# Foxhead-Studio/InsTaG

Measured on AMD Instinct MI355X. Metric: train-step frames/sec @512x512, 100k Gaussians, higher is better.
Workload: dtype f32; 1 GPU; C3: train_face step, 100k Gaussians + 6 grid encodes + UMF/PMF motion nets (DeepSpeech feats), 512x512, SH degree 1, image + attention map in one raster pass, L1+DSSIM, Adam; targets = uniform noise (SURVEY 8d); gaussians=100000, sh_degree=1, parallelism=dp1, ranks_reported_by_backend=1, execution=hipGraph replay, timing=one window of 1714 steps after 5 warm-up steps

## Files before the change

instag_amd/_lib.py:

```python
from __future__ import annotations

import ctypes as C
import os
import threading

from . import _cabi

HERE = os.path.dirname(os.path.abspath(__file__))
LIB_PATH = os.path.join(HERE, "lib", "libinstag_hip.so")

_lib = None
_lock = threading.Lock()

vp = C.c_void_p
i32 = C.c_int32
f32 = C.c_float

_STRUCTS, _PROTOTYPES, _CONSTANTS = _cabi.read()
globals().update((cls.__name__, cls) for cls in _STRUCTS.values())
EXPORTED_SYMBOLS = tuple(_PROTOTYPES)
ABI_VERSION = _CONSTANTS["INSTAG_ABI_VERSION"]
E_ARG = _CONSTANTS["INSTAG_E_ARG"]
FACE_LOSS = {k[len("INSTAG_FACE_LOSS_"):]: v for k, v in _CONSTANTS.items() if k.startswith("INSTAG_FACE_LOSS_")}

_WAV2VEC_STRUCTS, _WAV2VEC_PROTOTYPES, WAV2VEC = _cabi.read(os.path.join(os.path.dirname(_cabi.HEADER), "instag_wav2vec.h"))
globals().update((cls.__name__, cls) for cls in _WAV2VEC_STRUCTS.values())

_HUBERT_STRUCTS, _HUBERT_PROTOTYPES, HUBERT = _cabi.read(os.path.join(os.path.dirname(_cabi.HEADER), "instag_hubert.h"),
                                                         _WAV2VEC_STRUCTS)

_, _FRAME_CODE_WIDE_PROTOTYPES, _ = _cabi.read(os.path.join(os.path.dirname(_cabi.HEADER), "instag_frame_code_wide.h"))

_DEEPSPEECH_STRUCTS, _DEEPSPEECH_PROTOTYPES, DEEPSPEECH = _cabi.read(os.path.join(os.path.dirname(_cabi.HEADER),
                                                                              "instag_deepspeech.h"))
globals().update((cls.__name__, cls) for cls in _DEEPSPEECH_STRUCTS.values())

_LANDMARKS_STRUCTS, _LANDMARKS_PROTOTYPES, LANDMARKS = _cabi.read(os.path.join(os.path.dirname(_cabi.HEADER),
                                                                             "instag_landmarks.h"))
globals().update((cls.__name__, cls) for cls in _LANDMARKS_STRUCTS.values())

_FACE_DETECT_STRUCTS, _FACE_DETECT_PROTOTYPES, FACE_DETECT = _cabi.read(os.path.join(os.path.dirname(_cabi.HEADER),
                                                                                   "instag_face_detect.h"))
globals().update((cls.__name__, cls) for cls in _FACE_DETECT_STRUCTS.values())


_STREAMS = {}


def side_stream(device, tag, priority=0):
    import torch
    device = torch.device(device)
    index = device.index if device.index is not None else torch.cuda.current_device()
    key = (index, tag)
    s = _STREAMS.get(key)
    if s is None:
        taken = {v.cuda_stream for (d, _), v in _STREAMS.items() if d == index}
        for _ in range(64):
            s = torch.cuda.Stream(device=torch.device("cuda", index), priority=priority)
            if s.cuda_stream not in taken:
                break
        else:
            raise RuntimeError(f"no distinct HIP stream left for {tag!r} ({len(taken)} in use on device {index})")
        _STREAMS[key] = s
    return s


def capture_stream(device=None):
    import torch
    if device is None:
        device = torch.device("cuda", torch.cuda.current_device())
    return side_stream(device, "capture", priority=-1)


def warmup_stream(device):
    return side_stream(device, "warmup")

# ... 59 lines not shown


def may_fork(device=None) -> bool:
    import torch
    if _LEAF_STREAMS and any(torch.cuda.current_stream(device) == s for s in _LEAF_STREAMS):
        return False
    if not torch.cuda.is_current_stream_capturing():
        return True
    return _CAPTURE_ORIGIN is not None and torch.cuda.current_stream(device) == _CAPTURE_ORIGIN


_LEAF_STREAMS = []


def leaf_stream(stream):
    if all(stream != s for s in _LEAF_STREAMS):
        _LEAF_STREAMS.append(stream)


def lib():
    global _lib
    if _lib is not None:
        return _lib
    with _lock:
        if _lib is not None:
            return _lib
        if not os.path.exists(LIB_PATH):
            from . import build as _build
            _build.build(verbose=False)
        import torch
        handle = C.CDLL(LIB_PATH)
        for name, (res, args) in {**_PROTOTYPES, **_WAV2VEC_PROTOTYPES, **_HUBERT_PROTOTYPES,
                                  **_FRAME_CODE_WIDE_PROTOTYPES, **_DEEPSPEECH_PROTOTYPES,
                                  **_LANDMARKS_PROTOTYPES, **_FACE_DETECT_PROTOTYPES}.items():
            if not hasattr(handle, name):
                raise RuntimeError(f"{LIB_PATH} does not export {name}: rebuild it (python -m instag_amd.build)")
            fn = getattr(handle, name)
            fn.restype = res
            fn.argtypes = args
        if handle.instag_abi_version() != ABI_VERSION:
            raise RuntimeError(f"{LIB_PATH} has ABI version {handle.instag_abi_version()}, the bindings expect "
                               f"{ABI_VERSION}: rebuild it (python -c 'import __graft_entry__ as g; g.build()')")
        _lib = handle
    return _lib


def check(code: int, what: str = ""):
    if code != 0:
        msg = lib().instag_last_error().decode("utf-8", "replace")
        raise RuntimeError(f"{what}: {msg}" if what else msg)


def check_arg(code: int, what: str):
    if code != 0:
        msg = lib().instag_last_error().decode("utf-8", "replace")
        raise (ValueError if code == E_ARG else RuntimeError)(f"{what}: {msg}")


def workspace_bytes(nbytes: int) -> int:
    if nbytes == 0:
        raise ValueError(lib().instag_last_error().decode("utf-8", "replace"))
    return int(nbytes)


def ptr(t):
    return None if t is None else C.c_void_p(t.data_ptr())

# ... 5 lines not shown
```

instag_amd/csrc/raster_api.hip:

```cpp
#include <cstdio>
#include <cstdlib>
#include <cstring>

#include <mutex>
#include <vector>

#include "raster_internal.hpp"

namespace instag {

static thread_local std::string g_err;
void set_error(const std::string& msg) { g_err = msg; }

namespace {
struct ProfState {
  std::mutex mu;
  int mask = 0;
  struct Pair { hipEvent_t a, b; };
  std::vector<Pair> pending[INSTAG_PROF_KERNELS];
  double total_ms[INSTAG_PROF_KERNELS] = {0};
  int64_t launches[INSTAG_PROF_KERNELS] = {0};
  struct GraphPair { hipEvent_t a = nullptr, b = nullptr; int kernel = -1; bool closed = false; };
  std::vector<GraphPair> graph_pool;
  int graph_used = 0;
};
ProfState& prof() { static ProfState p; return p; }
}

static hipError_t record_external(hipEvent_t ev, hipStream_t stream) {
  static bool direct_ok = true;
  if (direct_ok) {
    if (hipEventRecordWithFlags(ev, stream, hipEventRecordExternal) == hipSuccess) return hipSuccess;
    (void)hipGetLastError();
    direct_ok = false;
  }
  hipStreamCaptureStatus st = hipStreamCaptureStatusNone;
  unsigned long long id = 0;
  hipGraph_t graph = nullptr;
  const hipGraphNode_t* deps = nullptr;
// ... 127 lines not shown
  L.tile_partials = o; o = align_up(o + (size_t)L.pre_blocks * WIDE_DIGITS * sizeof(uint32_t), 256);
  L.total = o;
  return L;
}

ImageLayout image_layout(int32_t H, int32_t W) {
  ImageLayout L;
  const size_t tiles = (size_t)div_up(W, TILE_X) * div_up(H, TILE_Y);
  const size_t P = (size_t)H * W;
  size_t o = 0;
  L.ranges = o; o = align_up(o + tiles * 2 * sizeof(int32_t), 256);
  L.n_contrib = o; o = align_up(o + P * sizeof(uint32_t), 256);
  L.final_T = o; o = align_up(o + P * sizeof(float), 256);
  L.tile_rounds = o; o = align_up(o + tiles * sizeof(uint32_t), 256);
  L.blend_mode = o; o = align_up(o + sizeof(uint32_t), 256);
  L.total = o;
  return L;
}

BinningLayout binning_layout(int64_t R, int32_t H, int32_t W) {
  BinningLayout L;
  const size_t r = (size_t)(R > 0 ? R : 1);
  const size_t tiles = (size_t)div_up(W, TILE_X) * div_up(H, TILE_Y);
  size_t o = 0;
  L.keys_unsorted = o; o = align_up(o + r * sizeof(uint32_t), 256);
  L.vals_unsorted = o; o = align_up(o + r * sizeof(uint32_t), 256);
  L.keys = o; o = align_up(o + r * sizeof(uint32_t), 256);
  L.vals = o; o = align_up(o + r * sizeof(uint32_t), 256);
  L.ktmp = o; o = align_up(o + r * sizeof(uint32_t), 256);
  L.vtmp = o; o = align_up(o + r * sizeof(uint32_t), 256);
  L.gid_unsorted = o; o = align_up(o + r * sizeof(uint32_t), 256);
  L.point_list = o; o = align_up(o + r * sizeof(uint32_t), 256);
  L.tsort_blocks = sort_blocks((uint32_t)r, SORT_IPT_TILE);
  const size_t wide_words = wide_tiles((int)tiles) ? (size_t)tile_pass_blocks((uint32_t)r) * 2 * ((tiles + 1) / 2) : 0;
  const size_t sort_words = 16 + std::max((size_t)3 * L.tsort_blocks * 256, wide_words);
  L.row_flag_stride = align_up(r, 16);
  L.seg_slots = r / SEG_LEN + tiles + 2;
  L.tsort_zero_words = sort_words + 4 + 2 * L.row_flag_stride / 4 + 8 * tiles + L.seg_slots;
  L.tsort_zero = o;
  L.seg_count = o + sort_words * sizeof(uint32_t);
  L.row_flag = L.seg_count + 4 * sizeof(uint32_t);
  L.fwd_sync = L.row_flag + 2 * L.row_flag_stride;
  L.seg_flag = L.fwd_sync + 8 * tiles * sizeof(uint32_t);
  o = align_up(o + L.tsort_zero_words * sizeof(uint32_t), 256);
  L.tsort_digit_base = o; o = align_up(o + (size_t)HIST_SLICES * 3 * 256 * sizeof(uint32_t), 256);
  L.tsort_partials = o; o = align_up(o + (size_t)1024 * 3 * 256 * sizeof(uint32_t), 256);
  L.sort_count = o; o = align_up(o + sizeof(uint32_t), 256);
  L.seg_queue = o; o = align_up(o + 2 * L.seg_slots * sizeof(uint32_t), 256);
  L.seg_state = o; o = align_up(o + L.seg_slots * SEG_FLOATS * TILE_PIX * sizeof(float), 256);
  L.total = o;
  return L;
}

static int validate(const instag_raster_args* a) {
  INSTAG_REQUIRE(a != nullptr, "raster args is NULL");
  INSTAG_REQUIRE(a->N >= 0, "N must be >= 0");
  INSTAG_REQUIRE(a->image_height > 0 && a->image_width > 0, "image size must be positive");
  INSTAG_REQUIRE(a->image_height <= 16368 && a->image_width <= 16368, "image larger than 16368 px not supported");
  INSTAG_REQUIRE((a->shs != nullptr) != (a->colors_precomp != nullptr),
                 "Please provide excatly one of either SHs or precomputed colors!");
  INSTAG_REQUIRE(((a->scales != nullptr && a->rotations != nullptr) && a->cov3Ds_precomp == nullptr) ||
                     ((a->scales == nullptr && a->rotations == nullptr) && a->cov3Ds_precomp != nullptr),
                 "Please provide exactly one of either scale/rotation pair or precomputed 3D covariance!");
  INSTAG_REQUIRE(a->E == 0 || a->E == 1, "extra_attrs: only 0 or 1 channel is supported");
  INSTAG_REQUIRE(a->sh_degree >= 0 && a->sh_degree <= 3, "sh_degree must be in [0,3]");
  if (a->shs) INSTAG_REQUIRE((a->sh_degree + 1) * (a->sh_degree + 1) <= a->M, "shs has fewer coefficients than sh_degree needs");
  INSTAG_REQUIRE(a->shs_rest == nullptr || (a->shs != nullptr && a->M >= 2), "shs_rest needs shs (the DC term) and M >= 2");
// ... 386 lines not shown
  const size_t n = std::min<size_t>((size_t)max_pairs, BL.seg_slots);
  if (n > 0) INSTAG_CHECK_HIP(hipMemcpyAsync(pairs, bb + BL.seg_queue, n * 2 * sizeof(uint32_t), hipMemcpyDeviceToDevice, s));
  if (blend_mode)
    INSTAG_CHECK_HIP(hipMemcpyAsync(blend_mode, ib + IL.blend_mode, sizeof(uint32_t), hipMemcpyDeviceToDevice, s));
  return INSTAG_OK;
}

int instag_raster_debug_export_flags(const void* geom, size_t geom_bytes, int32_t N, uint32_t* flags,
                                     instag_stream_t stream_) {
  const GeomLayout GL = geom_layout(N);
  INSTAG_REQUIRE(geom != nullptr && flags != nullptr, "debug_export_flags: NULL pointer");
  if (geom_bytes < GL.total) { set_error("geom buffer too small"); return INSTAG_E_SPACE; }
  if (N > 0)
    INSTAG_CHECK_HIP(hipMemcpyAsync(flags, (const char*)geom + GL.flags, (size_t)N * 4, hipMemcpyDeviceToDevice,
                                    (hipStream_t)stream_));
  return INSTAG_OK;
}

int instag_debug_depth_sort(const instag_raster_args* a, void* geom, size_t geom_bytes, uint64_t* stamps,
                            uint32_t* order_out, instag_stream_t stream_) {
  INSTAG_REQUIRE(a != nullptr && a->N > 0, "debug_depth_sort: N must be positive");
  const GeomLayout L = geom_layout(a->N);
  if (geom_bytes < L.total) { set_error("geom buffer too small"); return INSTAG_E_SPACE; }
  const Camera c = make_camera(a);
  if (int e = depth_sort(c, a, (char*)geom, L, (hipStream_t)stream_, stamps)) return e;
  if (order_out)
    INSTAG_CHECK_HIP(hipMemcpyAsync(order_out, (char*)geom + L.order, (size_t)a->N * 4, hipMemcpyDeviceToDevice,
                                    (hipStream_t)stream_));
  return INSTAG_OK;
}

uint32_t instag_debug_depth_sort_blocks(int32_t N) { return geom_layout(N).dsort_blocks; }

int instag_raster_sort_stalls(uint32_t* count, int32_t synchronize, instag_stream_t stream_) {
  INSTAG_REQUIRE(count != nullptr, "sort_stalls: count is NULL");
  return read_sort_stalls(count, (hipStream_t)stream_, synchronize != 0);
}

int instag_raster_sort_stalls_clear(instag_stream_t stream_) { return clear_sort_stalls((hipStream_t)stream_); }

int instag_debug_scan_stall_probe(instag_stream_t stream_) {
  hipStream_t s = (hipStream_t)stream_;
  constexpr int N = 8;
  uint32_t host[3 * N];
  for (int i = 0; i < N; ++i) { host[i] = (uint32_t)i; host[N + i] = 1u; host[2 * N + i] = 0u; }
  const uint64_t state_host[4] = {1ull, 0ull, 0ull, 0ull};
  char* dev = nullptr;
  INSTAG_CHECK_HIP(hipMalloc((void**)&dev, sizeof(host) + sizeof(state_host)));
  hipError_t err = hipMemcpyAsync(dev, host, sizeof(host), hipMemcpyHostToDevice, s);
  if (err == hipSuccess) err = hipMemcpyAsync(dev + sizeof(host), state_host, sizeof(state_host), hipMemcpyHostToDevice, s);
  int rc = INSTAG_OK;
  if (err == hipSuccess)
    rc = launch_scan_counts(N, (const uint32_t*)dev, (const uint32_t*)dev + N, (uint32_t*)dev + 2 * N,
                            (uint64_t*)(dev + sizeof(host)), s);
  if (err == hipSuccess) err = hipStreamSynchronize(s);
  (void)hipFree(dev);
  if (err != hipSuccess) { set_error(std::string("scan_stall_probe: ") + hipGetErrorString(err)); return INSTAG_E_HIP; }
  return rc;
}

int instag_prof_enable(int mask) {
  ProfState& p = prof();
  std::lock_guard<std::mutex> lk(p.mu);
  p.mask = mask;
  return INSTAG_OK;
}
// ... 92 lines not shown
```

instag_amd/csrc/raster_internal.hpp:

```cpp
#pragma once
#include "common.hpp"

namespace instag {

struct Camera {
  int32_t N, M, sh_degree, E, H, W;
  float tanfovx, tanfovy, focal_x, focal_y, scale_modifier;
  int32_t grid_x, grid_y;
  const float *bg, *view, *proj, *campos;
};

Camera make_camera(const instag_raster_args* a);

constexpr int WIDE_DIGITS = 2048;
inline bool wide_tiles(int tiles) { return tiles < (1 << 11) - 1; }
struct WideTileCounts {
  const uint32_t* partials;
  int n_partials;
  uint32_t *total, *dropped;
};

struct TilePasses {
  int npass, bits_per, nbits[3];
};
// ... 8 lines not shown
}

int launch_preprocess(const Camera& c, const instag_raster_args* a, float* rec2d, float* cov3d,
                      uint32_t* tiles_touched, uint32_t* flags, float* cull_thr, int32_t* radii,
                      uint32_t* tile_partials, uint32_t* zero_words, uint32_t n_zero_words, hipStream_t s);
uint32_t preprocess_blocks(int32_t N);
uint32_t depth_key_blocks(int32_t N);
int launch_depth_keys(const Camera& c, const float* means3D, uint32_t* depth_key, uint32_t* partials,
                      uint32_t* zero_words, uint32_t n_zero_words, hipStream_t s);
int launch_export_keys(int64_t R, const uint32_t* tile_keys, const uint32_t* point_list, const float* rec2d,
                       uint64_t* keys64, bool packed, hipStream_t s);
uint32_t duplicate_blocks(int32_t N);
int launch_duplicate(const Camera& c, float* rec2d, const uint32_t* order,
                     const uint32_t* point_offsets, const uint32_t* flags, const float* cull_thr, uint32_t* keys,
                     uint32_t* vals, uint32_t* gid_unsorted, uint32_t capacity, int32_t* ranges,
                     bool packed, int32_t* status, uint32_t* sort_count, const TilePasses& tp, uint32_t* partials,
                     uint32_t* zero_words, uint32_t n_zero_words, const WideTileCounts* wide, hipStream_t s);
int launch_ranges(int64_t R, const uint32_t* count_ptr, const uint32_t* keys_sorted, uint32_t* slots_sorted,
                  const uint32_t* gid_unsorted, uint32_t* point_list, int32_t* ranges, uint32_t ntiles, bool packed,
                  hipStream_t s);

constexpr int SORT_IPT_DEPTH = 4;
constexpr int SORT_IPT_TILE = 8;
constexpr int HIST_SLICES = 8;
uint32_t sort_blocks(uint32_t count_max, int ipt);
int launch_radix_pass(int ipt, bool has_values, bool write_keys, const uint32_t* keys_in, uint32_t* keys_out,
                      const uint32_t* vals_in, uint32_t* vals_out, const uint32_t* count_ptr, uint32_t count_max,
                      int shift, int nbits, const uint32_t* hist, int n_hist, int hist_stride, uint32_t* ticket,
                      uint32_t* lookback, hipStream_t s, uint64_t* stamps = nullptr);
int read_sort_stalls(uint32_t* host_out, hipStream_t s, bool synchronize);
int clear_sort_stalls(hipStream_t s);
uint32_t* sort_stalls_device_ptr();
int launch_hist_reduce(const uint32_t* partials, int nblk, int npass, int slices, uint32_t* out, hipStream_t s);
uint32_t tile_pass_blocks(uint32_t count_max);
int launch_tile_pass(const uint32_t* keys_in, const uint32_t* gid_unsorted, uint32_t* keys_out, uint32_t* slots_out,
                     uint32_t* point_list, int32_t* ranges, const uint32_t* count_ptr, uint32_t count_max, int tiles,
                     const uint32_t* tile_total, const uint32_t* tile_dropped, uint32_t* ticket, uint64_t* lookback,
                     hipStream_t s, uint64_t* stamps = nullptr);
int launch_scan_counts(int N, const uint32_t* order, const uint32_t* tiles_touched, uint32_t* point_offsets,
                       uint64_t* state, hipStream_t s);

constexpr int PACK_SHIFT = 21;
inline bool use_packed_keys(int64_t R, int tiles) { return R < ((int64_t)1 << PACK_SHIFT) && tiles < (1 << 11) - 1; }

int launch_blend_forward(const Camera& c, const int32_t* ranges, const uint32_t* point_list,
                         const float* rec2d, uint32_t* n_contrib, float* final_T, float* out_color,
                         float* out_depth, float* out_normal, float* out_alpha, float* out_extra,
                         const float* aux_colors, float* out_aux, uint32_t* seg_queue, uint32_t* seg_count,
                         float* seg_state, uint32_t* tile_rounds, uint32_t* tile_sync ,
                         uint32_t* seg_flag , uint32_t* walk_hints ,
                         int64_t instances, bool colour_only ,
                         uint32_t* blend_mode ,
                         hipStream_t s);
int launch_blend_backward(const Camera& c, const int32_t* ranges, const uint32_t* point_list,
                          const uint32_t* slot_list, const float* rec2d, const uint32_t* n_contrib, const float* final_T,
                          const float* dL_dcolor, const float* dL_ddepth, const float* dL_dnormal,
                          const float* dL_dalpha, const float* dL_dextra, float* inst_grad,
                          const float* color_override, const float* aux_colors, const float* dL_daux, int aux_mode,
                          const uint32_t* seg_queue, const uint32_t* seg_count, const float* seg_state,
                          const uint32_t* tile_rounds, uint32_t seg_slots, uint8_t* row_flag,
                          const uint32_t* blend_mode, hipStream_t s);

int launch_preprocess_backward(const Camera& c, const instag_raster_args* a, const float* rec2d,
                               const float* cov3d, const uint32_t* tiles_touched, const uint32_t* flags,
                               const int32_t* radii, const float* inst_grad, uint8_t* row_flag, uint32_t capacity,
                               float* dL_dmeans3D,
                               float* dL_dmeans2D, float* dL_dshs, float* dL_dcolors,
                               float* dL_dopacities, float* dL_dscales, float* dL_drotations,
                               float* dL_dcov3D, float* dL_dextra, float* dL_dshs_rest, float* dL_daux_colors,
                               hipStream_t s);
int launch_aux_backward_reduce(const Camera& c, const float* rec2d, const uint32_t* tiles_touched, const int32_t* radii,
// ... 5 lines not shown
```

instag_amd/csrc/raster_sort.hip:

```cpp
#include "device_math.hpp"
#include "raster_internal.hpp"

namespace instag {
namespace {

constexpr int SORT_THREADS = 256;
constexpr int PASS_THREADS = 1024;
constexpr int RADIX = 256;
constexpr int SPIN_LIMIT = 1 << 21;
constexpr int LB_CHUNK = 8;
constexpr uint32_t LB_PARTIAL = 1u << 30, LB_COMPLETE = 2u << 30, LB_FLAGS = 3u << 30, LB_VALUE = ~LB_FLAGS;

__device__ uint32_t g_sort_stalls = 0;

__device__ __forceinline__ uint32_t ld_agent(const uint32_t* p) {
  return __hip_atomic_load(p, __ATOMIC_RELAXED, __HIP_MEMORY_SCOPE_AGENT);
}
__device__ __forceinline__ void st_agent(uint32_t* p, uint32_t v) {
  __hip_atomic_store(p, v, __ATOMIC_RELAXED, __HIP_MEMORY_SCOPE_AGENT);
}
__device__ __forceinline__ uint64_t ld_agent64(const uint64_t* p) {
  return __hip_atomic_load(p, __ATOMIC_RELAXED, __HIP_MEMORY_SCOPE_AGENT);
}
__device__ __forceinline__ void st_agent64(uint64_t* p, uint64_t v) {
// ... 191 lines not shown
      const uint32_t dst = s_gbase[(kv >> shift) & mask] + p;
      if (WRITE_KEYS) keys_out[dst] = kv;
      if (HAS_VALUES) vals_out[dst] = s_vals[p];
    }
  }
  INSTAG_STAMP(5);
#undef INSTAG_STAMP
}

__device__ __forceinline__ uint32_t block_exclusive_scan_1024(uint32_t v, uint32_t* s_w, uint32_t* total) {
  constexpr int WAVES = PASS_THREADS / 64;
  const int lane = threadIdx.x & 63, wave = threadIdx.x >> 6;
  uint32_t inc = v;
#pragma unroll
  for (int o = 1; o < 64; o <<= 1) {
    const uint32_t t = __shfl_up(inc, o);
    if (lane >= o) inc += t;
  }
  if (lane == 63) s_w[wave] = inc;
  __syncthreads();
  uint32_t base = 0, sum = 0;
#pragma unroll
  for (int w = 0; w < WAVES; ++w) {
    const uint32_t x = s_w[w];
    base += (w < wave) ? x : 0u;
    sum += x;
  }
  *total = sum;
  return base + inc - v;
}

constexpr int TILE_WIDE_IPT = 5;
constexpr int TILE_WIDE = PASS_THREADS * TILE_WIDE_IPT;

__global__ void __launch_bounds__(PASS_THREADS)
tile_pass_kernel(const uint32_t* __restrict__ keys_in, const uint32_t* __restrict__ gid_unsorted,
                 uint32_t* __restrict__ keys_out, uint32_t* __restrict__ slots_out, uint32_t* __restrict__ point_list,
                 int32_t* __restrict__ ranges, const uint32_t* __restrict__ count_ptr, uint32_t count_max, int ntiles,
                 int nbits, const uint32_t* __restrict__ tile_total, const uint32_t* __restrict__ tile_dropped,
                 uint32_t* __restrict__ ticket, uint64_t* __restrict__ lookback, int lb_stride,
                 uint64_t* __restrict__ stamps) {
  constexpr int IPT = TILE_WIDE_IPT;
  constexpr int WAVES = PASS_THREADS / 64;
  constexpr int PAIRS = WIDE_DIGITS / 2;
  static_assert(PAIRS == PASS_THREADS, "one thread per digit pair");
  static_assert(2 * TILE_WIDE < 65536, "16-bit digit offsets");
#define INSTAG_STAMP(k) do { if (stamps != nullptr && threadIdx.x == 0) stamps[(size_t)s_bid * 8 + (k)] = __builtin_amdgcn_s_memrealtime(); } while (0)
  __shared__ uint32_t s_cnt[WAVES][PAIRS];
  __shared__ uint32_t s_gbase[WIDE_DIGITS];
  __shared__ uint32_t s_keys[TILE_WIDE];
  __shared__ uint32_t s_gid[TILE_WIDE];
  __shared__ uint32_t s_w[WAVES], s_w2[WAVES];
  __shared__ uint32_t s_bid;
  const int tid = threadIdx.x, lane = tid & 63, wave = tid >> 6;
  for (int k = tid; k < WAVES * PAIRS; k += PASS_THREADS) (&s_cnt[0][0])[k] = 0u;
  if (tid == 0) s_bid = atomicAdd(ticket, 1u);
  __syncthreads();
  const uint32_t bid = s_bid;
  INSTAG_STAMP(0);
  uint32_t count = count_ptr ? *count_ptr : count_max;
  count = min(count, count_max);
  const uint64_t base = (uint64_t)bid * TILE_WIDE;
  if (base >= count) return;
  const uint32_t valid = (uint32_t)min((uint64_t)TILE_WIDE, (uint64_t)count - base);

  uint32_t key[IPT], gid[IPT], rank[IPT];
#pragma unroll
  for (int i = 0; i < IPT; ++i) {
    const uint32_t idx = min((uint32_t)wave * (64 * IPT) + i * 64 + lane, valid - 1u);
    key[i] = keys_in[base + idx];
    gid[i] = gid_unsorted[base + idx];
  }
  const int d0 = 2 * tid;
  uint32_t gt0 = 0, gt1 = 0;
  if (d0 < ntiles) gt0 = tile_total[d0] - tile_dropped[d0];
  if (d0 + 1 < ntiles) gt1 = tile_total[d0 + 1] - tile_dropped[d0 + 1];
  INSTAG_STAMP(1);
  const uint64_t lt_mask = (1ull << lane) - 1ull;
  uint16_t* cnt16 = reinterpret_cast<uint16_t*>(&s_cnt[wave][0]);
#pragma unroll
  for (int i = 0; i < IPT; ++i) {
    const uint32_t idx = (uint32_t)wave * (64 * IPT) + i * 64 + lane;
    const bool ok = idx < valid;
    const uint32_t d = key[i] >> PACK_SHIFT;
    uint64_t peers = __builtin_amdgcn_ballot_w64(ok);
    for (int b = 0; b < nbits; ++b) {
      const bool bit = (d >> b) & 1u;
      const uint64_t m = __builtin_amdgcn_ballot_w64(bit);
      peers &= bit ? m : ~m;
    }
    const uint32_t prev = ok ? cnt16[d] : 0u;
    if (ok && lane == __builtin_ctzll(peers)) cnt16[d] = (uint16_t)(prev + (uint32_t)__builtin_popcountll(peers));
    rank[i] = prev + (uint32_t)__builtin_popcountll(peers & lt_mask);
  }
  __syncthreads();
  INSTAG_STAMP(2);
  {
    uint32_t wc[WAVES], c0 = 0, c1 = 0;
#pragma unroll
    for (int w = 0; w < WAVES; ++w) {
      wc[w] = s_cnt[w][tid];
      const uint32_t lo = wc[w] & 0xFFFFu, hi = wc[w] >> 16;
      wc[w] = c0 | (c1 << 16);
      c0 += lo;
      c1 += hi;
    }
    uint32_t unused = 0;
    const uint32_t dstart0 = block_exclusive_scan_1024(c0 + c1, s_w, &unused);
    const uint32_t dstart1 = dstart0 + c0;
    uint32_t tsum = 0;
    const uint32_t gstart0 = block_exclusive_scan_1024(gt0 + gt1, s_w2, &tsum);
    const uint32_t gstart1 = gstart0 + gt0;
#pragma unroll
    for (int w = 0; w < WAVES; ++w) s_cnt[w][tid] = wc[w] + (dstart0 | (dstart1 << 16));
    if (tid == 0 && tsum != count) atomicAdd(&g_sort_stalls, 1u);
    if (bid == 0) {
      if (d0 < ntiles) {
        ranges[2 * d0] = gt0 ? (int32_t)gstart0 : 0;
        ranges[2 * d0 + 1] = gt0 ? (int32_t)(gstart0 + gt0) : 0;
      }
      if (d0 + 1 < ntiles) {
        ranges[2 * d0 + 2] = gt1 ? (int32_t)gstart1 : 0;
        ranges[2 * d0 + 3] = gt1 ? (int32_t)(gstart1 + gt1) : 0;
      }
    }
    INSTAG_STAMP(3);
    uint32_t excl0 = 0, excl1 = 0;
    bool done0 = gt0 == 0, done1 = gt1 == 0;
    if (!(done0 && done1)) {
      uint64_t* mine = lookback + (size_t)bid * lb_stride + tid;
      st_agent64(mine, (uint64_t)(LB_PARTIAL | c0) | ((uint64_t)(LB_PARTIAL | c1) << 32));
      uint32_t b = bid;
      while (b > 0 && !(done0 && done1)) {
        uint64_t st[LB_CHUNK];
#pragma unroll
        for (int j = 0; j < LB_CHUNK; ++j)
          st[j] = (uint32_t)j < b ? ld_agent64(lookback + (size_t)(b - 1 - j) * lb_stride + tid) : 0ull;
#pragma unroll
        for (int j = 0; j < LB_CHUNK; ++j) {
          if ((uint32_t)j < b && !(done0 && done1)) {
            const uint64_t* p = lookback + (size_t)(b - 1 - j) * lb_stride + tid;
            auto waiting = [&](uint64_t v) {
              return (!done0 && ((uint32_t)v & LB_FLAGS) == 0u) || (!done1 && ((uint32_t)(v >> 32) & LB_FLAGS) == 0u);
            };
            for (int polls = 0; waiting(st[j]) && polls < SPIN_LIMIT; ++polls) {
              __builtin_amdgcn_s_sleep(1);
              st[j] = ld_agent64(p);
            }
            if (waiting(st[j])) atomicAdd(&g_sort_stalls, 1u);
            const uint32_t w0 = (uint32_t)st[j], w1 = (uint32_t)(st[j] >> 32);
            if (!done0) {
              excl0 += w0 & LB_VALUE;
              done0 = (w0 & LB_FLAGS) == LB_COMPLETE;
            }
            if (!done1) {
              excl1 += w1 & LB_VALUE;
              done1 = (w1 & LB_FLAGS) == LB_COMPLETE;
            }
          }
        }
        b = b > (uint32_t)LB_CHUNK ? b - LB_CHUNK : 0u;
      }
      st_agent64(mine, (uint64_t)(LB_COMPLETE | (excl0 + c0)) | ((uint64_t)(LB_COMPLETE | (excl1 + c1)) << 32));
    }
    s_gbase[d0] = gstart0 + excl0 - dstart0;
    s_gbase[d0 + 1] = gstart1 + excl1 - dstart1;
  }
  __syncthreads();
  INSTAG_STAMP(4);
#pragma unroll
  for (int i = 0; i < IPT; ++i) {
    const uint32_t idx = (uint32_t)wave * (64 * IPT) + i * 64 + lane;
    if (idx < valid) {
      const uint32_t p = (uint32_t)cnt16[key[i] >> PACK_SHIFT] + rank[i];
      s_keys[p] = key[i];
      s_gid[p] = gid[i];
    }
  }
  __syncthreads();
#pragma unroll
  for (int k = 0; k < IPT; ++k) {
    const uint32_t p = (uint32_t)k * PASS_THREADS + tid;
    if (p < valid) {
      const uint32_t kv = s_keys[p];
      const uint32_t dst = s_gbase[kv >> PACK_SHIFT] + p;
      if (dst < count) {
        keys_out[dst] = kv;
        slots_out[dst] = kv & ((1u << PACK_SHIFT) - 1u);
        point_list[dst] = s_gid[p];
      }
    }
  }
  INSTAG_STAMP(5);
#undef INSTAG_STAMP
}

// ... 84 lines not shown
                  int n_hist, int hist_stride, uint32_t* ticket, uint32_t* lookback, uint64_t* stamps, hipStream_t s) {
  const uint32_t blocks = div_up<uint32_t>(count_max, PASS_THREADS * IPT);
  if (blocks == 0) return INSTAG_OK;
  radix_pass_kernel<IPT, HAS_VALUES, WRITE_KEYS><<<blocks, PASS_THREADS, 0, s>>>(
      keys_in, keys_out, vals_in, vals_out, count_ptr, count_max, shift, nbits, hist, n_hist, hist_stride, ticket,
      lookback, stamps);
  INSTAG_CHECK_LAUNCH();
  return INSTAG_OK;
}

}

uint32_t sort_blocks(uint32_t count_max, int ipt) { return div_up<uint32_t>(count_max, PASS_THREADS * ipt); }

int launch_radix_pass(int ipt, bool has_values, bool write_keys, const uint32_t* keys_in, uint32_t* keys_out,
                      const uint32_t* vals_in, uint32_t* vals_out, const uint32_t* count_ptr, uint32_t count_max,
                      int shift, int nbits, const uint32_t* hist, int n_hist, int hist_stride, uint32_t* ticket,
                      uint32_t* lookback, hipStream_t s, uint64_t* stamps) {
#define INSTAG_PASS(I, V, K)                                                                                         \
  if (ipt == I && has_values == V && write_keys == K)                                                                \
    return launch_pass_t<I, V, K>(keys_in, keys_out, vals_in, vals_out, count_ptr, count_max, shift, nbits,          \
                                  hist, n_hist, hist_stride, ticket, lookback, stamps, s);
  INSTAG_PASS(SORT_IPT_DEPTH, true, true)
  INSTAG_PASS(SORT_IPT_DEPTH, true, false)
  INSTAG_PASS(SORT_IPT_TILE, false, true)
  INSTAG_PASS(SORT_IPT_TILE, true, true)
#undef INSTAG_PASS
  set_error("launch_radix_pass: unsupported variant");
  return INSTAG_E_ARG;
}

uint32_t tile_pass_blocks(uint32_t count_max) { return div_up<uint32_t>(count_max, TILE_WIDE); }

int launch_tile_pass(const uint32_t* keys_in, const uint32_t* gid_unsorted, uint32_t* keys_out, uint32_t* slots_out,
                     uint32_t* point_list, int32_t* ranges, const uint32_t* count_ptr, uint32_t count_max, int tiles,
                     const uint32_t* tile_total, const uint32_t* tile_dropped, uint32_t* ticket, uint64_t* lookback,
                     hipStream_t s, uint64_t* stamps) {
  if (!wide_tiles(tiles) || tiles <= 0) {
    set_error("launch_tile_pass: too many tiles for the one-pass sort");
    return INSTAG_E_ARG;
  }
  const uint32_t blocks = tile_pass_blocks(count_max);
  if (blocks == 0) return INSTAG_OK;
  int nbits = 0;
  while ((1 << nbits) < tiles) ++nbits;
  tile_pass_kernel<<<blocks, PASS_THREADS, 0, s>>>(keys_in, gid_unsorted, keys_out, slots_out, point_list, ranges,
                                                   count_ptr, count_max, tiles, nbits, tile_total, tile_dropped,
                                                   ticket, lookback, (tiles + 1) / 2, stamps);
  INSTAG_CHECK_LAUNCH();
  return INSTAG_OK;
}

int launch_hist_reduce(const uint32_t* partials, int nblk, int npass, int slices, uint32_t* out, hipStream_t s) {
  if (npass <= 0 || nblk <= 0) return INSTAG_OK;
  hist_reduce_kernel<<<dim3(npass, slices), SORT_THREADS, 0, s>>>(partials, nblk, npass, div_up(nblk, slices), out);
  INSTAG_CHECK_LAUNCH();
  return INSTAG_OK;
}

int read_sort_stalls(uint32_t* host_out, hipStream_t s, bool synchronize) {
  INSTAG_CHECK_HIP(hipMemcpyFromSymbolAsync(host_out, HIP_SYMBOL(g_sort_stalls), sizeof(uint32_t), 0,
                                            hipMemcpyDeviceToHost, s));
  if (synchronize) INSTAG_CHECK_HIP(hipStreamSynchronize(s));
  return INSTAG_OK;
}

uint32_t* sort_stalls_device_ptr() {
  static uint32_t* cached[64] = {};
  int dev = 0;
  if (hipGetDevice(&dev) != hipSuccess || dev < 0 || dev >= 64) return nullptr;
  if (cached[dev] == nullptr) {
    void* p = nullptr;
    if (hipGetSymbolAddress(&p, HIP_SYMBOL(g_sort_stalls)) != hipSuccess) return nullptr;
    cached[dev] = (uint32_t*)p;
  }
  return cached[dev];
}

int clear_sort_stalls(hipStream_t s) {
  const uint32_t zero = 0;
  INSTAG_CHECK_HIP(hipMemcpyToSymbolAsync(HIP_SYMBOL(g_sort_stalls), &zero, sizeof(uint32_t), 0, hipMemcpyHostToDevice, s));
// ... 15 lines not shown
```

instag_amd/diff_gauss.py:

```python
from __future__ import annotations

import ctypes as C
from typing import NamedTuple, Optional

import torch
import torch.nn as nn

from . import _keepalive, _lib
from ._lib import RasterArgs, check, ptr


class GaussianRasterizationSettings(NamedTuple):
    image_height: int
    image_width: int
    tanfovx: float
    tanfovy: float
    bg: torch.Tensor
    scale_modifier: float
    viewmatrix: torch.Tensor
    projmatrix: torch.Tensor
    sh_degree: int
    campos: torch.Tensor
    prefiltered: bool
    debug: bool
# ... 55 lines not shown
                raise RuntimeError(f"rasterizer binning: {int(self._host_stalls[0])} sort / scan look-back(s) gave up "
                                   "waiting for their predecessor; the affected steps rendered wrong tile lists")
            result = [(k, int(st[k, 2])) for k in range(len(self.capacities)) if int(st[k, 1]) != 0]
            self._event = None
        if self._event is None:
            if self._host is None:
                self._host = torch.zeros(len(self.capacities), 4, dtype=torch.int32).pin_memory()
                self._host_stalls = torch.zeros(1, dtype=torch.int32).pin_memory()
            self._host.copy_(self._all, non_blocking=True)
            check(_lib.lib().instag_raster_sort_stalls(C.c_void_p(self._host_stalls.data_ptr()), 0,
                                                       _lib.current_stream()), "sort_stalls")
            self._event = torch.cuda.Event()
            self._event.record()
        return result

    def needed(self):
        return [int(v) for v in self._all.cpu()[:, 0]]

    def peak(self):
        return [int(v) for v in self._all.cpu()[:, 2]]

    def clear(self):
        self._all.zero_()
        self._event = None


def sort_stalls(clear: bool = False) -> int:
    L = _lib.lib()
    n = C.c_uint32(0)
    check(L.instag_raster_sort_stalls(C.byref(n), 1, _lib.current_stream()), "sort_stalls")
    if clear and n.value:
        check(L.instag_raster_sort_stalls_clear(_lib.current_stream()), "sort_stalls_clear")
    return int(n.value)


_CAPACITY_PLAN = None


def set_capacity_plan(plan):
    global _CAPACITY_PLAN
    _CAPACITY_PLAN = plan


class _State:
    __slots__ = ("args", "keep", "geom", "binning", "image", "R", "radii", "N", "H", "W", "E", "M", "aux", "split_sh",
                 "geometry")


def _make_args(s: GaussianRasterizationSettings, means3D, shs, colors, opac, scales, rots, cov3D, extra):
    N = means3D.shape[0]
    shs_rest = None
    if isinstance(shs, (tuple, list)):
        shs, shs_rest = shs
        if shs_rest.shape[1] == 0:
            shs_rest = None
    M = 0 if shs is None else shs.shape[1] + (0 if shs_rest is None else shs_rest.shape[1])
    E = 0 if extra is None else (extra.shape[1] if extra.dim() > 1 else 1)
    bg, view, proj, campos = _f32c(s.bg), _f32c(s.viewmatrix), _f32c(s.projmatrix), _f32c(s.campos)
    _require_cuda(bg=bg, viewmatrix=view, projmatrix=proj, campos=campos)
    a = RasterArgs()
    a.N, a.M, a.sh_degree, a.E = N, M, int(s.sh_degree), E
    a.image_height, a.image_width = int(s.image_height), int(s.image_width)
    a.tanfovx, a.tanfovy, a.scale_modifier = float(s.tanfovx), float(s.tanfovy), float(s.scale_modifier)
    a.prefiltered, a.debug = int(bool(s.prefiltered)), int(bool(s.debug))
    a.single_stream = 0 if _lib.may_fork(means3D.device) else 1
    a.bg, a.viewmatrix, a.projmatrix, a.campos = ptr(bg), ptr(view), ptr(proj), ptr(campos)
# ... 329 lines not shown
```

Before: 1059 frames/s.

## Replace decoupled look-back in tile sort with two-level grouped block aggregates

The one-pass tile sort kernel no longer walks back block by block through decoupled look-back with partial/complete flags. Blocks are now grouped in sets of 16. Each block publishes its per-tile counts, and the last block of a group also publishes the group aggregate. Every block then sums its in-group predecessors plus all earlier group aggregates, and the aggregate publication is moved ahead of the local scan so other blocks can proceed sooner. This is meant to bound the serial look-back chain and cut polling latency, at the cost of more loads per block and an extra aggregate array in the workspace. A debug entry point and Python wrapper are added for testing with other group sizes.

New measurement: 1063 frames/s (median of 6 runs). No clear change (+0.4%).

```diff
diff --git a/include/instag_raster_debug.h b/include/instag_raster_debug.h
--- /dev/null
+++ b/include/instag_raster_debug.h
@@ -0,0 +1,21 @@
+#ifndef INSTAG_RASTER_DEBUG_H
+#define INSTAG_RASTER_DEBUG_H
+
+#include "instag_hip.h"
+
+#ifdef __cplusplus
+extern "C" {
+#endif
+
+uint32_t instag_debug_tile_pass_blocks(uint32_t count_max);
+size_t instag_debug_tile_pass_workspace_bytes(uint32_t count_max, int32_t ntiles, int32_t group);
+int instag_debug_tile_pass(const uint32_t* keys_in, const uint32_t* gid_in, const uint32_t* count, uint32_t count_max,
+                           int32_t ntiles, const uint32_t* tile_total, int32_t group, void* workspace,
+                           size_t workspace_bytes, uint32_t* keys_out, uint32_t* slots, uint32_t* point_list,
+                           int32_t* ranges, uint64_t* stamps, instag_stream_t stream);
+
+#ifdef __cplusplus
+}
+#endif
+
+#endif
diff --git a/instag_amd/_lib.py b/instag_amd/_lib.py
--- a/instag_amd/_lib.py
+++ b/instag_amd/_lib.py
@@ -42,6 +42,8 @@
 _FACE_DETECT_STRUCTS, _FACE_DETECT_PROTOTYPES, FACE_DETECT = _cabi.read(os.path.join(os.path.dirname(_cabi.HEADER),
                                                                                    "instag_face_detect.h"))
 globals().update((cls.__name__, cls) for cls in _FACE_DETECT_STRUCTS.values())
+
+_, _RASTER_DEBUG_PROTOTYPES, _ = _cabi.read(os.path.join(os.path.dirname(_cabi.HEADER), "instag_raster_debug.h"))
 
 
 _STREAMS = {}
@@ -167,7 +169,8 @@
         handle = C.CDLL(LIB_PATH)
         for name, (res, args) in {**_PROTOTYPES, **_WAV2VEC_PROTOTYPES, **_HUBERT_PROTOTYPES,
                                   **_FRAME_CODE_WIDE_PROTOTYPES, **_DEEPSPEECH_PROTOTYPES,
-                                  **_LANDMARKS_PROTOTYPES, **_FACE_DETECT_PROTOTYPES}.items():
+                                  **_LANDMARKS_PROTOTYPES, **_FACE_DETECT_PROTOTYPES,
+                                  **_RASTER_DEBUG_PROTOTYPES}.items():
             if not hasattr(handle, name):
                 raise RuntimeError(f"{LIB_PATH} does not export {name}: rebuild it (python -m instag_amd.build)")
             fn = getattr(handle, name)
diff --git a/instag_amd/csrc/raster_api.hip b/instag_amd/csrc/raster_api.hip
--- a/instag_amd/csrc/raster_api.hip
+++ b/instag_amd/csrc/raster_api.hip
@@ -5,6 +5,7 @@
 #include <mutex>
 #include <vector>
 
+#include "instag_raster_debug.h"
 #include "raster_internal.hpp"
 
 namespace instag {
@@ -198,7 +199,7 @@
   L.gid_unsorted = o; o = align_up(o + r * sizeof(uint32_t), 256);
   L.point_list = o; o = align_up(o + r * sizeof(uint32_t), 256);
   L.tsort_blocks = sort_blocks((uint32_t)r, SORT_IPT_TILE);
-  const size_t wide_words = wide_tiles((int)tiles) ? (size_t)tile_pass_blocks((uint32_t)r) * 2 * ((tiles + 1) / 2) : 0;
+  const size_t wide_words = wide_tiles((int)tiles) ? tile_pass_lookback_words((uint32_t)r, (int)tiles) : 0;
   const size_t sort_words = 16 + std::max((size_t)3 * L.tsort_blocks * 256, wide_words);
   L.row_flag_stride = align_up(r, 16);
   L.seg_slots = r / SEG_LEN + tiles + 2;
@@ -651,6 +652,42 @@
 
 uint32_t instag_debug_depth_sort_blocks(int32_t N) { return geom_layout(N).dsort_blocks; }
 
+static int tile_pass_group_shift(int32_t group) {
+  if (group == 0) return TILE_LB_GROUP_SHIFT;
+  for (int sh = 1; sh <= 6; ++sh)
+    if (group == (1 << sh)) return sh;
+  return -1;
+}
+
+uint32_t instag_debug_tile_pass_blocks(uint32_t count_max) { return tile_pass_blocks(count_max); }
+
+size_t instag_debug_tile_pass_workspace_bytes(uint32_t count_max, int32_t ntiles, int32_t group) {
+  const int gshift = tile_pass_group_shift(group);
+  if (gshift < 0 || ntiles <= 0 || !wide_tiles(ntiles) || !use_packed_keys(count_max, ntiles)) {
+    set_error("debug_tile_pass: group must be 0 or a power of two in [2, 64], 0 < ntiles < 2047, count_max < 2^21");
+    return 0;
+  }
+  return (16 + tile_pass_lookback_words(count_max, ntiles, gshift) + WIDE_DIGITS) * sizeof(uint32_t);
+}
+
+int instag_debug_tile_pass(const uint32_t* keys_in, const uint32_t* gid_in, const uint32_t* count, uint32_t count_max,
+                           int32_t ntiles, const uint32_t* tile_total, int32_t group, void* workspace,
+                           size_t workspace_bytes, uint32_t* keys_out, uint32_t* slots, uint32_t* point_list,
+                           int32_t* ranges, uint64_t* stamps, instag_stream_t stream_) {
+  hipStream_t s = (hipStream_t)stream_;
+  const size_t need = instag_debug_tile_pass_workspace_bytes(count_max, ntiles, group);
+  if (need == 0) return INSTAG_E_ARG;
+  INSTAG_REQUIRE(keys_in && gid_in && count && tile_total && workspace && keys_out && slots && point_list && ranges,
+                 "debug_tile_pass: NULL pointer");
+  if (workspace_bytes < need) { set_error("debug_tile_pass: workspace too small"); return INSTAG_E_SPACE; }
+  const int gshift = tile_pass_group_shift(group);
+  uint32_t* zero = (uint32_t*)workspace;
+  const uint32_t* dropped = zero + 16 + tile_pass_lookback_words(count_max, ntiles, gshift);
+  INSTAG_CHECK_HIP(hipMemsetAsync(workspace, 0, need, s));
+  return launch_tile_pass(keys_in, gid_in, keys_out, slots, point_list, ranges, count, count_max, ntiles, tile_total,
+                          dropped, zero, (uint64_t*)(zero + 16), s, gshift, stamps);
+}
+
 int instag_raster_sort_stalls(uint32_t* count, int32_t synchronize, instag_stream_t stream_) {
   INSTAG_REQUIRE(count != nullptr, "sort_stalls: count is NULL");
   return read_sort_stalls(count, (hipStream_t)stream_, synchronize != 0);
diff --git a/instag_amd/csrc/raster_internal.hpp b/instag_amd/csrc/raster_internal.hpp
--- a/instag_amd/csrc/raster_internal.hpp
+++ b/instag_amd/csrc/raster_internal.hpp
@@ -64,11 +64,13 @@
 int clear_sort_stalls(hipStream_t s);
 uint32_t* sort_stalls_device_ptr();
 int launch_hist_reduce(const uint32_t* partials, int nblk, int npass, int slices, uint32_t* out, hipStream_t s);
+constexpr int TILE_LB_GROUP_SHIFT = 4;
 uint32_t tile_pass_blocks(uint32_t count_max);
+size_t tile_pass_lookback_words(uint32_t count_max, int tiles, int gshift = TILE_LB_GROUP_SHIFT);
 int launch_tile_pass(const uint32_t* keys_in, const uint32_t* gid_unsorted, uint32_t* keys_out, uint32_t* slots_out,
                      uint32_t* point_list, int32_t* ranges, const uint32_t* count_ptr, uint32_t count_max, int tiles,
                      const uint32_t* tile_total, const uint32_t* tile_dropped, uint32_t* ticket, uint64_t* lookback,
-                     hipStream_t s, uint64_t* stamps = nullptr);
+                     hipStream_t s, int gshift = TILE_LB_GROUP_SHIFT, uint64_t* stamps = nullptr);
 int launch_scan_counts(int N, const uint32_t* order, const uint32_t* tiles_touched, uint32_t* point_offsets,
                        uint64_t* state, hipStream_t s);
 
diff --git a/instag_amd/csrc/raster_sort.hip b/instag_amd/csrc/raster_sort.hip
--- a/instag_amd/csrc/raster_sort.hip
+++ b/instag_amd/csrc/raster_sort.hip
@@ -247,13 +247,14 @@
 
 constexpr int TILE_WIDE_IPT = 5;
 constexpr int TILE_WIDE = PASS_THREADS * TILE_WIDE_IPT;
+constexpr int LB_WIDE = 16;
 
 __global__ void __launch_bounds__(PASS_THREADS)
 tile_pass_kernel(const uint32_t* __restrict__ keys_in, const uint32_t* __restrict__ gid_unsorted,
                  uint32_t* __restrict__ keys_out, uint32_t* __restrict__ slots_out, uint32_t* __restrict__ point_list,
                  int32_t* __restrict__ ranges, const uint32_t* __restrict__ count_ptr, uint32_t count_max, int ntiles,
                  int nbits, const uint32_t* __restrict__ tile_total, const uint32_t* __restrict__ tile_dropped,
-                 uint32_t* __restrict__ ticket, uint64_t* __restrict__ lookback, int lb_stride,
+                 uint32_t* __restrict__ ticket, uint64_t* __restrict__ lookback, int lb_stride, int gshift,
                  uint64_t* __restrict__ stamps) {
   constexpr int IPT = TILE_WIDE_IPT;
   constexpr int WAVES = PASS_THREADS / 64;
@@ -320,6 +321,41 @@
       c0 += lo;
       c1 += hi;
     }
+    const bool look = (gt0 | gt1) != 0u;
+    const uint32_t grp = bid >> gshift, first = grp << gshift, in_grp = bid - first;
+    const bool closes_group = in_grp + 1u == (1u << gshift);
+    const uint64_t* counts = lookback + tid;
+    uint64_t* aggs = lookback + (size_t)gridDim.x * lb_stride + tid;
+    uint32_t excl0 = 0, excl1 = 0;
+    auto settle = [&](uint64_t v, const uint64_t* p) {
+      for (int polls = 0; ((uint32_t)v & LB_FLAGS) == 0u && polls < SPIN_LIMIT; ++polls) {
+        __builtin_amdgcn_s_sleep(1);
+        v = ld_agent64(p);
+      }
+      if (((uint32_t)v & LB_FLAGS) == 0u) atomicAdd(&g_sort_stalls, 1u);
+      excl0 += (uint32_t)v & LB_VALUE;
+      excl1 += (uint32_t)(v >> 32) & LB_VALUE;
+    };
+    auto add_group_counts = [&]() {
+      for (uint32_t i0 = 0; i0 < in_grp; i0 += LB_WIDE) {
+        uint64_t st[LB_WIDE];
+#pragma unroll
+        for (int k = 0; k < LB_WIDE; ++k)
+          st[k] = i0 + k < in_grp ? ld_agent64(counts + (size_t)(first + i0 + k) * lb_stride) : 0ull;
+#pragma unroll
+        for (int k = 0; k < LB_WIDE; ++k)
+          if (i0 + k < in_grp) settle(st[k], counts + (size_t)(first + i0 + k) * lb_stride);
+      }
+    };
+    if (look) {
+      st_agent64(lookback + (size_t)bid * lb_stride + tid,
+                 (uint64_t)(LB_PARTIAL | c0) | ((uint64_t)(LB_PARTIAL | c1) << 32));
+      if (closes_group) {
+        add_group_counts();
+        st_agent64(aggs + (size_t)grp * lb_stride,
+                   (uint64_t)(LB_PARTIAL | (excl0 + c0)) | ((uint64_t)(LB_PARTIAL | (excl1 + c1)) << 32));
+      }
+    }
     uint32_t unused = 0;
     const uint32_t dstart0 = block_exclusive_scan_1024(c0 + c1, s_w, &unused);
     const uint32_t dstart1 = dstart0 + c0;
@@ -340,43 +376,21 @@
       }
     }
     INSTAG_STAMP(3);
-    uint32_t excl0 = 0, excl1 = 0;
-    bool done0 = gt0 == 0, done1 = gt1 == 0;
-    if (!(done0 && done1)) {
-      uint64_t* mine = lookback + (size_t)bid * lb_stride + tid;
-      st_agent64(mine, (uint64_t)(LB_PARTIAL | c0) | ((uint64_t)(LB_PARTIAL | c1) << 32));
-      uint32_t b = bid;
-      while (b > 0 && !(done0 && done1)) {
-        uint64_t st[LB_CHUNK];
-#pragma unroll
-        for (int j = 0; j < LB_CHUNK; ++j)
-          st[j] = (uint32_t)j < b ? ld_agent64(lookback + (size_t)(b - 1 - j) * lb_stride + tid) : 0ull;
-#pragma unroll
-        for (int j = 0; j < LB_CHUNK; ++j) {
-          if ((uint32_t)j < b && !(done0 && done1)) {
-            const uint64_t* p = lookback + (size_t)(b - 1 - j) * lb_stride + tid;
-            auto waiting = [&](uint64_t v) {
-              return (!done0 && ((uint32_t)v & LB_FLAGS) == 0u) || (!done1 && ((uint32_t)(v >> 32) & LB_FLAGS) == 0u);
-            };
-            for (int polls = 0; waiting(st[j]) && polls < SPIN_LIMIT; ++polls) {
-              __builtin_amdgcn_s_sleep(1);
-              st[j] = ld_agent64(p);
-            }
-            if (waiting(st[j])) atomicAdd(&g_sort_stalls, 1u);
-            const uint32_t w0 = (uint32_t)st[j], w1 = (uint32_t)(st[j] >> 32);
-            if (!done0) {
-              excl0 += w0 & LB_VALUE;
-              done0 = (w0 & LB_FLAGS) == LB_COMPLETE;
-            }
-            if (!done1) {
-              excl1 += w1 & LB_VALUE;
-              done1 = (w1 & LB_FLAGS) == LB_COMPLETE;
-            }
-          }
-        }
-        b = b > (uint32_t)LB_CHUNK ? b - LB_CHUNK : 0u;
-      }
-      st_agent64(mine, (uint64_t)(LB_COMPLETE | (excl0 + c0)) | ((uint64_t)(LB_COMPLETE | (excl1 + c1)) << 32));
+    if (look) {
+      uint64_t ag[LB_WIDE];
+#pragma unroll
+      for (int k = 0; k < LB_WIDE; ++k) ag[k] = (uint32_t)k < grp ? ld_agent64(aggs + (size_t)k * lb_stride) : 0ull;
+      if (!closes_group) add_group_counts();
+#pragma unroll
+      for (int k = 0; k < LB_WIDE; ++k)
+        if ((uint32_t)k < grp) settle(ag[k], aggs + (size_t)k * lb_stride);
+      for (uint32_t i0 = LB_WIDE; i0 < grp; i0 += LB_WIDE) {
+#pragma unroll
+        for (int k = 0; k < LB_WIDE; ++k) ag[k] = i0 + k < grp ? ld_agent64(aggs + (size_t)(i0 + k) * lb_stride) : 0ull;
+#pragma unroll
+        for (int k = 0; k < LB_WIDE; ++k)
+          if (i0 + k < grp) settle(ag[k], aggs + (size_t)(i0 + k) * lb_stride);
+      }
     }
     s_gbase[d0] = gstart0 + excl0 - dstart0;
     s_gbase[d0 + 1] = gstart1 + excl1 - dstart1;
@@ -527,12 +541,21 @@
 
 uint32_t tile_pass_blocks(uint32_t count_max) { return div_up<uint32_t>(count_max, TILE_WIDE); }
 
+size_t tile_pass_lookback_words(uint32_t count_max, int tiles, int gshift) {
+  const size_t blocks = tile_pass_blocks(count_max);
+  return (blocks + (blocks >> gshift)) * 2 * (size_t)((tiles + 1) / 2);
+}
+
 int launch_tile_pass(const uint32_t* keys_in, const uint32_t* gid_unsorted, uint32_t* keys_out, uint32_t* slots_out,
                      uint32_t* point_list, int32_t* ranges, const uint32_t* count_ptr, uint32_t count_max, int tiles,
                      const uint32_t* tile_total, const uint32_t* tile_dropped, uint32_t* ticket, uint64_t* lookback,
-                     hipStream_t s, uint64_t* stamps) {
+                     hipStream_t s, int gshift, uint64_t* stamps) {
   if (!wide_tiles(tiles) || tiles <= 0) {
     set_error("launch_tile_pass: too many tiles for the one-pass sort");
+    return INSTAG_E_ARG;
+  }
+  if (gshift < 1 || gshift > 6) {
+    set_error("launch_tile_pass: look-back groups are 2 to 64 blocks");
     return INSTAG_E_ARG;
   }
   const uint32_t blocks = tile_pass_blocks(count_max);
@@ -541,7 +564,7 @@
   while ((1 << nbits) < tiles) ++nbits;
   tile_pass_kernel<<<blocks, PASS_THREADS, 0, s>>>(keys_in, gid_unsorted, keys_out, slots_out, point_list, ranges,
                                                    count_ptr, count_max, tiles, nbits, tile_total, tile_dropped,
-                                                   ticket, lookback, (tiles + 1) / 2, stamps);
+                                                   ticket, lookback, (tiles + 1) / 2, gshift, stamps);
   INSTAG_CHECK_LAUNCH();
   return INSTAG_OK;
 }
diff --git a/instag_amd/diff_gauss.py b/instag_amd/diff_gauss.py
--- a/instag_amd/diff_gauss.py
+++ b/instag_amd/diff_gauss.py
@@ -111,6 +111,30 @@
     if clear and n.value:
         check(L.instag_raster_sort_stalls_clear(_lib.current_stream()), "sort_stalls_clear")
     return int(n.value)
+
+
+def debug_tile_pass(keys, count, ntiles, gid=None, group=0, stamps=False):
+    L = _lib.lib()
+    dev = keys.device
+    count_max = int(keys.numel())
+    n = min(int(count), count_max)
+    keys32 = (keys.to(torch.int64) & 0xFFFFFFFF).to(torch.uint32).contiguous()
+    if gid is None:
+        gid = (torch.arange(count_max, device=dev, dtype=torch.int64) * 2654435761) & 0x7FFFFFFF
+    gid32 = gid.to(torch.int64).to(torch.uint32).contiguous()
+    totals = torch.bincount(keys.to(torch.int64)[:n] >> 21, minlength=ntiles).to(torch.uint32)
+    nbytes = _lib.workspace_bytes(L.instag_debug_tile_pass_workspace_bytes(count_max, ntiles, group))
+    work = torch.empty(nbytes, dtype=torch.uint8, device=dev)
+    cnt = torch.tensor([int(count)], dtype=torch.int64).to(torch.uint32).to(dev)
+    out = [torch.zeros(max(count_max, 1), dtype=torch.uint32, device=dev) for _ in range(3)]
+    ranges = torch.full((ntiles, 2), -1, dtype=torch.int32, device=dev)
+    st = torch.zeros(L.instag_debug_tile_pass_blocks(count_max), 8, dtype=torch.int64, device=dev) if stamps else None
+    check(L.instag_debug_tile_pass(_lib.ptr(keys32), _lib.ptr(gid32), _lib.ptr(cnt), count_max, ntiles,
+                                   _lib.ptr(totals), group, _lib.ptr(work), nbytes, _lib.ptr(out[0]), _lib.ptr(out[1]),
+                                   _lib.ptr(out[2]), _lib.ptr(ranges), _lib.ptr(st), _lib.current_stream()),
+          "debug_tile_pass")
+    res = tuple(t[:count_max] for t in out) + (ranges,)
+    return res + (st,) if stamps else res
 
 
 _CAPACITY_PLAN = None
```
